# isl-org/adaptive-surface-reconstruction

Hardware: AMD Instinct MI355X
Metric: input points/sec to signed implicit values (higher is better)
Workload: dtype f32 via bf16x3 (24-bit operands, f32 accumulate)

## Files before the change

### adaptive-surface-reconstruction_amd/csrc/asr_api.hip

```cpp
#include <cmath>
#include <cstdlib>
#include <cstring>

#include <algorithm>
#include <functional>
#include <future>
#include <mutex>
#include <thread>

#include "asr_common.h"
#include "asr_uset.h"

#define ASR_ROW_GROUP_SEGMENT (ctx->opt.row_segment > 0 ? ctx->opt.row_segment : (i64)524288)
#define CTX_GUARD(ctx)                                                  \
    if (!(ctx)) return ASR_HIP_EINVAL;                                  \
    (ctx)->err.clear();                                                 \
    if (hipSetDevice((ctx)->device) != hipSuccess) {                    \
        (ctx)->err = "hipSetDevice failed for the context's device";   \
        return ASR_HIP_EHIP;                                            \
    }

namespace {
struct OptEntry {
    const char* name;
    const char* env;
    i64 AsrOptions::*field;
};
const OptEntry k_options[] = {
        {"sconv_min_blocks", "ASR_SCONV_MIN_BLOCKS", &AsrOptions::sconv_min_blocks},
        {"sconv_wide_min", "ASR_SCONV_WIDE_MIN", &AsrOptions::sconv_wide_min},
        {"row_segment", "ASR_ROW_SEGMENT", &AsrOptions::row_segment},
        {"row_lpt", "ASR_ROW_LPT", &AsrOptions::row_lpt},
        {"row_ranked", "ASR_ROW_RANKED", &AsrOptions::row_ranked},
        {"sconv_plan", "ASR_SCONV_PLAN", &AsrOptions::sconv_plan},
        {"plan_arena", "ASR_PLAN_ARENA", &AsrOptions::plan_arena},
        {"sconv16_min_blocks", "ASR_SCONV16_MIN_BLOCKS", &AsrOptions::sconv16_min_blocks},
        {"knn_cells", "ASR_KNN_CELLS", &AsrOptions::knn_cells},
        {"knn_deep", "ASR_KNN_DEEP", &AsrOptions::knn_deep},
        {"search_hash_level", "ASR_SEARCH_HASH_LEVEL", &AsrOptions::search_hash_level},
        {"overlap", "ASR_OVERLAP", &AsrOptions::overlap},
        {"build_search", "ASR_BUILD_SEARCH", &AsrOptions::build_search},
        {"cconv_valu", "ASR_CCONV_VALU", &AsrOptions::cconv_valu},
        {"search_half", "ASR_SEARCH_HALF", &AsrOptions::search_half},
        {"search_priority", "ASR_SEARCH_PRIORITY", &AsrOptions::search_priority},
        {"shard_timing", "ASR_SHARD_TIMING", &AsrOptions::shard_timing},
        {"shard_geometry", "ASR_SHARD_GEOMETRY", &AsrOptions::shard_geometry},
        {"early_sort", "ASR_EARLY_SORT", &AsrOptions::early_sort},
        {"early_cells", "ASR_EARLY_CELLS", &AsrOptions::early_cells},
        {"sconv_split_rows", "ASR_SCONV_SPLIT_ROWS", &AsrOptions::sconv_split_rows},
        {"sconv_split_min_rows", "ASR_SCONV_SPLIT_MIN_ROWS", &AsrOptions::sconv_split_min_rows},
        {"arena_cap_mb", "ASR_ARENA_CAP_MB", &AsrOptions::arena_cap_mb},
        {"inject_failure", "ASR_INJECT_FAILURE", &AsrOptions::inject_failure},
};
void apply_arena_cap(asr_hip_context* ctx) {
    const size_t cap = ctx->opt.arena_cap_mb > 0 ? (size_t)ctx->opt.arena_cap_mb << 20 : 0;
    for (asr_hip_context* c : {ctx, ctx->aux})
// ... 930 lines not shown
            const i64* rs;
            const int32_t* perm;
            i64 rows;
            int K;
        };
        std::vector<Job> jobs;
        for (int i = 0; i < ASR_NUM_GRIDS; ++i) {
            GridDev& g = ctx->grids[i];
            jobs.push_back({g.nidx, g.nkidx, g.nrs, g.perm_nb, g.v, 55});
            if (i + 1 < ASR_NUM_GRIDS) {
                GridDev& c = ctx->grids[i + 1];
                jobs.push_back({g.up_idx, g.up_kidx, g.up_rs, g.perm_up, g.v, 9});
                jobs.push_back({g.down_idx, g.down_kidx, g.down_rs, g.perm_down, c.v, 9});
            }
        }
        std::vector<asr_conv_plan> plans(jobs.size());
        for (size_t j = 0; j < jobs.size(); ++j) {
            plans[j].nidx = jobs[j].idx;
            plans[j].kidx = jobs[j].kidx;
            plans[j].rs = jobs[j].rs;
            plans[j].perm = jobs[j].perm;
            plans[j].num_out = jobs[j].rows;
            plans[j].K = jobs[j].K;
        }
        const int rc = asr_geom_conv_plan_batch(on, on->persist, plans.data(), (int)plans.size());
        if (rc != ASR_HIP_OK) {
            if (on != ctx) ctx->err = on->err;
            return rc;
        }
        for (size_t j = 0; j < jobs.size(); ++j) ctx->conv_plans[jobs[j].rs] = plans[j];
    }
    return ASR_HIP_OK;
}

__global__ void k_gather_queries(const int32_t* rows, i64 nq, const float* centers, const float* sizes, const u64* keys,
                                 float* qc, float* qs, u64* qk) {
    const i64 i = blockIdx.x * (i64)blockDim.x + threadIdx.x;
    if (i >= nq) return;
    const i64 r = rows[i];
    qc[3 * i] = centers[3 * r];
    qc[3 * i + 1] = centers[3 * r + 1];
    qc[3 * i + 2] = centers[3 * r + 2];
    qs[i] = sizes[r];
    qk[i] = keys[r];
}
__global__ void k_scatter_rows(const float* src, const int32_t* rows, i64 nq, int c, float* dst) {
// ... 667 lines not shown
```

### adaptive-surface-reconstruction_amd/csrc/asr_common.h

```cpp
#pragma once
#include <hip/hip_runtime.h>

#include <cstdint>
#include <cstdio>
#include <map>
#include <string>
#include <tuple>
#include <vector>

#include "../../include/asr_hip.h"

typedef uint64_t u64;
typedef int64_t i64;
typedef uint32_t u32;

struct Arena {
    struct Slab {
        char* base;
        size_t size, used;
    };
    std::vector<Slab> slabs;
    size_t min_slab = size_t(256) << 20;
    size_t cap = 0;

// ... 48 lines not shown
    i64* nrs = nullptr;
    int32_t* up_idx = nullptr;
    uint8_t* up_kidx = nullptr;
    i64* up_rs = nullptr;
    int32_t* down_idx = nullptr;
    uint8_t* down_kidx = nullptr;
    i64* down_rs = nullptr;
    int32_t* perm_nb = nullptr;
    int32_t* perm_up = nullptr;
    int32_t* perm_down = nullptr;
};

struct AsrOptions {
    i64 sconv_min_blocks = 2816;
    i64 sconv16_min_blocks = 1024;
    i64 sconv_wide_min = 2048;
    i64 row_segment = 524288;
    i64 search_hash_level = -1;
    i64 knn_deep = 1;
    i64 knn_cells = 1;
    i64 plan_arena = 0;
    i64 sconv_plan = 1;
    i64 row_ranked = 1;
    i64 row_lpt = 1;
    i64 overlap = 1;
    i64 cconv_valu = 0;
    i64 build_search = 1;
    i64 shard_geometry = -1;
    i64 shard_timing = 0;
    i64 search_priority = 2;
    i64 search_half = 1;
    i64 early_cells = 1;
    i64 early_sort = 1;
    i64 arena_cap_mb = 0;
    i64 inject_failure = 0;
    i64 sconv_split_min_rows = 2048;
    i64 sconv_split_rows = 32768;
};

struct asr_conv_plan_view {
    const uint4* hdr;
    const int32_t* pool;
    i64 groups;
    unsigned pool_bytes;
};
struct asr_conv_plan {
    uint4* hdr = nullptr;
    int32_t* pool = nullptr;
    i64 groups = 0, groups_pad = 0, blocks = 0;
    i64* offs = nullptr;
    const int32_t* nidx = nullptr;
    const uint8_t* kidx = nullptr;
    const i64* rs = nullptr;
    const int32_t* perm = nullptr;
    i64 num_out = 0;
    int K = 0;
    bool usable() const { return hdr && blocks * 64 < (i64(1) << 32) - 65536; }
    asr_conv_plan_view view() const { return {hdr, pool, groups, (unsigned)(blocks * 64)}; }
};

struct AsrPointIndex {
    bool valid = false;
    const float* pts = nullptr;
    const float* radii = nullptr;
    i64 n = 0;
    int lsort = 0;
    float4* sorted = nullptr;
    int32_t* ids = nullptr;
    int32_t* rank = nullptr;
    float* srad = nullptr;
    u64* codes = nullptr;
    u64* tab_keys = nullptr;
    u64 tab_mask = 0;
    int32_t* tab_start = nullptr;
    int32_t* tab_end = nullptr;
    int tab_lmin = 0, tab_lmax = -1, tab_lhash = 0, tab_grow = 0;
};

struct asr_hip_context {
// ... 214 lines not shown
int asr_geom_grid_neighbors_count(asr_hip_context* ctx, const u64* keys, i64 v, const int32_t* rows, i64 nrows, i64* rs,
                                  i64* num_pairs);
int asr_geom_grid_neighbors_fill(asr_hip_context* ctx, const u64* keys, i64 v, const int32_t* rows, i64 nrows,
                                 const i64* rs, int32_t* idx, uint8_t* kidx);
struct asr_nb_job {
    const u64* keys;
    i64 v;
    i64* rs;
    int32_t* idx;
    uint8_t* kidx;
    i64 p;
    const int32_t* owner = nullptr;
    int me = 0;
};
int asr_geom_neighbors_build_batch(asr_hip_context* ctx, Arena& out_arena, asr_nb_job* jobs, int n);
int asr_geom_row_groups(asr_hip_context* ctx, const uint8_t* kidx, const i64* rs, i64 v, i64 seg,
                        int32_t* perm_out, int kbits);
struct asr_row_group_job {
    const uint8_t* kidx;
    const i64* rs;
    i64 v;
    int kbits;
    int32_t* perm_out;
};
int asr_geom_row_groups_batch(asr_hip_context* ctx, const asr_row_group_job* jobs, int n, i64 seg);
int asr_geom_coarsen_count(asr_hip_context* ctx, const u64* keys, i64 v, i64* v_out);
int asr_geom_coarsen_fill(asr_hip_context* ctx, const u64* keys, i64 v, u64* out_keys, i64 v_out,
                          int32_t* up_idx, uint8_t* up_kidx, i64* up_rs);
int asr_geom_coarsen_build(asr_hip_context* ctx, Arena& keep, const u64* keys, i64 v, u64** out_keys, i64* v_out,
                           int32_t** up_idx, uint8_t** up_kidx, i64** up_rs, int32_t** down_idx, uint8_t** down_kidx,
                           i64** down_rs);
int asr_geom_voxel_info(asr_hip_context* ctx, const asr_octree_frame* frame, const u64* keys,
                        i64 v, float* centers, float* sizes);
int asr_geom_radius_count(asr_hip_context* ctx, const asr_octree_frame* frame, const float* pts,
                          i64 n, const float* centers, const float* sizes, i64 v, i64* rs,
                          i64* num_pairs, Arena* keep = nullptr, const float* radii = nullptr,
                          const u64* voxel_keys = nullptr, int lmin_hint = -1, int lmax_hint = -1,
                          const AsrPointIndex* pre = nullptr);

int asr_geom_radius_fill(asr_hip_context* ctx, const float* pts, const float* radii, i64 n,
                         const float* centers, const float* sizes, i64 v, const i64* rs,
                         int32_t* idx, float* dist, float* compat, int32_t* spos = nullptr,
                         const float4** sorted_out = nullptr);
int asr_geom_radius_neighbor_count(asr_hip_context* ctx, const asr_octree_frame* frame, const float* pts,
                                   const float* radii, i64 n, i64* counts_out);
int asr_geom_attributes_at(asr_hip_context* ctx, const asr_octree_frame* frame, const float* pts, const float* radii, i64 n,
                           const float* attr, int c, const float* positions, const float* sizes, i64 m, int max_widen,
                           float min_weight, float fill, float* out, float* weight_out, int8_t* widen_out);
// ... 60 lines not shown
```

### adaptive-surface-reconstruction_amd/csrc/asr_geom.hip

```cpp
#include <cstdlib>
#include <cstring>
#include <algorithm>
#include <rocprim/rocprim.hpp>

#include "asr_common.h"
#include "asr_prim.h"

namespace {
using namespace asr_prim;

constexpr int BLK = 256;

struct HashTab {
    u64* keys;
    int32_t* vals;
    u64 mask;
};

struct TabProbe {
    u64 bucket, step, low, bmask;
    __device__ inline u64 slot() const { return ((bucket & bmask) << 6) | low; }
    __device__ inline void next() { bucket += step; }
};
__device__ inline TabProbe tab_probe(const HashTab& t, u64 key) {
// ... 551 lines not shown
}
__global__ void k_iota64(i64* out, i64 n) {
    i64 i = blockIdx.x * (i64)blockDim.x + threadIdx.x;
    if (i < n) out[i] = i;
}

__global__ void k_voxel_info(asr_octree_frame f, const u64* keys, i64 v, float* centers,
                             float* sizes) {
    i64 i = blockIdx.x * (i64)blockDim.x + threadIdx.x;
    if (i >= v) return;
    int x, y, z, lev;
    asr_key_coord(keys[i], x, y, z, lev);
    int s = ASR_MAX_LEVEL - lev;
    double half = 0.5 * (double)(u64(1) << s);
    double vs = (double)f.voxel_size[ASR_MAX_LEVEL];
    if (centers) {
        centers[3 * i + 0] = (float)((((x << s) - f.offset[0]) + half) * vs);
        centers[3 * i + 1] = (float)((((y << s) - f.offset[1]) + half) * vs);
        centers[3 * i + 2] = (float)((((z << s) - f.offset[2]) + half) * vs);
    }
    if (sizes) sizes[i] = f.voxel_size[lev];
}

__global__ void k_point_codes(asr_octree_frame f, const float* pts, i64 n, u64* codes,
                              int32_t* ids, int* cnt) {
    i64 i = blockIdx.x * (i64)blockDim.x + threadIdx.x;
    if (i >= n) return;
    if (!(isfinite(pts[3 * i]) && isfinite(pts[3 * i + 1]) && isfinite(pts[3 * i + 2]))) cnt[11] = 1;
    int x, y, z;
    frame_coord(f, pts[3 * i], pts[3 * i + 1], pts[3 * i + 2], ASR_MAX_LEVEL, x, y, z);
    const int lim = (1 << ASR_MAX_LEVEL) - 1;
    x = min(max(x, 0), lim);
    y = min(max(y, 0), lim);
    z = min(max(z, 0), lim);
    codes[i] = asr_morton3d((u64)x, (u64)y, (u64)z);
    ids[i] = (int32_t)i;
}
__global__ void k_gather_points(const float* pts, const int32_t* ids, i64 n, float4* sorted, int32_t* rank,
                                const float* radii = nullptr, float* srad = nullptr) {
    i64 i = blockIdx.x * (i64)blockDim.x + threadIdx.x;
    if (i >= n) return;
    int32_t id = ids[i];
    sorted[i] = make_float4(pts[3 * (i64)id], pts[3 * (i64)id + 1], pts[3 * (i64)id + 2],
                            __int_as_float(id));
    if (rank) rank[id] = (int32_t)i;
    if (srad) srad[i] = radii[id];
}
__global__ void k_gather_radii(const float* radii, const int32_t* ids, i64 n, float* out) {
    i64 i = blockIdx.x * (i64)blockDim.x + threadIdx.x;
    if (i < n) out[i] = radii[ids[i]];
}
__device__ inline int query_level(const asr_octree_frame& f, float r) {
    int lev = 0;
    while (lev < ASR_MAX_LEVEL && f.voxel_size[lev + 1] >= r) ++lev;
    return lev;
}
__global__ __launch_bounds__(256) void k_query_levels(asr_octree_frame f, const float* sizes, i64 v, int* cnt) {
    __shared__ int s_lo[4], s_hi[4];
    int lo = ASR_MAX_LEVEL, hi = 0;
// ... 1171 lines not shown
        __syncthreads();
        const int m = min(2048, n - base);
        for (int e = 0; e < m; ++e) rank += s_key[e] < mine;
    }
    if (i < n) t.vals[slot_of[i]] = rank;
}
__global__ void k_rg_keys_ranked(RowGroupBatch b, i64 seg, const u64* masks, HashTab t, unsigned* keys, int32_t* ids,
                                 int rank_bits) {
    const i64 e = blockIdx.x * (i64)blockDim.x + threadIdx.x;
    if (e >= b.base[b.n]) return;
    const int j = rg_job_of(b, e);
    const i64 r = e - b.base[j];
    unsigned key;
    if (r < b.v[j]) {
        const int rank = tab_find(t, (masks[e] >> 1) + 1);
        key = ((unsigned)j << (6 + rank_bits)) | ((unsigned)(r / seg) << rank_bits) | (unsigned)rank;
    } else {
        key = ((unsigned)j << (6 + rank_bits)) | (63u << rank_bits) | ((1u << rank_bits) - 1u);
    }
    keys[e] = key;
    ids[e] = (int32_t)e;
}

__device__ inline u64 dev_morton_add(u64 a, u64 b) {
    const u64 M = 0x9249249249249249ull;
    u64 c = ((a | ~M) + (b & M)) & M;
    c |= ((a | ~(M << 1)) + (b & (M << 1))) & (M << 1);
    c |= ((a | ~(M << 2)) + (b & (M << 2))) & (M << 2);
    return c;
}
__device__ inline u64 dev_morton_sub(u64 a, u64 b) {
    const u64 M = 0x9249249249249249ull;
    u64 c = ((a & M) - (b & M)) & M;
    c |= ((a & (M << 1)) - (b & (M << 1))) & (M << 1);
    c |= ((a & (M << 2)) - (b & (M << 2))) & (M << 2);
    return c;
}
__device__ inline int node_lookup(const HashTab& t, u64 key) {
    TabProbe pr = tab_probe(t, key);
    for (u64 probe = 0; probe <= pr.bmask; ++probe, pr.next()) {
        const u64 slot = pr.slot();
        const u64 cur = t.keys[slot];
        if (cur == key) return t.vals[slot];
        if (cur == 0) return -2;
    }
    return -2;
// ... 412 lines not shown
    }
    if (perm_m != perm_out) {
        const i64 nc = (v + 127) / 128;
        int32_t* ckey = arena_alloc<int32_t>(ctx->scratch, nc);
        int32_t* ckey_s = arena_alloc<int32_t>(ctx->scratch, nc);
        int32_t* cid = arena_alloc<int32_t>(ctx->scratch, nc);
        int32_t* cid_s = arena_alloc<int32_t>(ctx->scratch, nc);
        if (!ckey || !ckey_s || !cid || !cid_s) ASR_FAIL(ctx, ASR_HIP_EHIP, "arena allocation failed");
        int32_t* tcost = arena_alloc<int32_t>(ctx->scratch, 2 * nc);
        if (!tcost) ASR_FAIL(ctx, ASR_HIP_EHIP, "arena allocation failed");
        k_tile_cost<<<grid_for(((v + 63) / 64) * 64, BLK), BLK, 0, ctx->stream>>>(perm_m, masks, v, tcost);
        ASR_CHECK_LAUNCH(ctx);
        k_chunk_key<<<grid_for(nc, BLK), BLK, 0, ctx->stream>>>(tcost, v, seg, ckey, cid);
        ASR_CHECK_LAUNCH(ctx);
        ASR_TRY((sort_pairs<int32_t, int32_t>(ctx, ctx->scratch, ckey, ckey_s, cid, cid_s, nc,
                                              7 + bits_for((v + seg - 1) / seg + 1))));
        k_chunk_apply<<<grid_for(v, BLK), BLK, 0, ctx->stream>>>(perm_m, cid_s, v, perm_out);
        ASR_CHECK_LAUNCH(ctx);
    }
    return ASR_HIP_OK;
}

static int rg_batch_run(asr_hip_context* ctx, const asr_row_group_job* jobs, int n, i64 seg, int mask_bits);
static int rg_batch_run_ranked(asr_hip_context* ctx, const asr_row_group_job* jobs, int n, i64 seg, bool* done);
int asr_geom_row_groups_batch(asr_hip_context* ctx, const asr_row_group_job* jobs, int n, i64 seg) {
    if (seg < 128) seg = 128;
    bool fits = n <= RG_MAX_JOBS && seg % 128 == 0;
    for (int j = 0; j < n && fits; ++j) fits = jobs[j].v / seg < 63 && jobs[j].v < (i64(1) << 31);
    if (!fits) {
        for (int j = 0; j < n; ++j)
            ASR_TRY(asr_geom_row_groups(ctx, jobs[j].kidx, jobs[j].rs, jobs[j].v, seg, jobs[j].perm_out, jobs[j].kbits));
        return ASR_HIP_OK;
    }
    if (ctx->opt.row_ranked) {
        bool done = false;
        ASR_TRY(rg_batch_run_ranked(ctx, jobs, n, seg, &done));
        if (done) return ASR_HIP_OK;
    }
    std::vector<asr_row_group_job> small_jobs, wide_jobs;
    for (int j = 0; j < n; ++j) (jobs[j].kbits <= 10 ? small_jobs : wide_jobs).push_back(jobs[j]);
    if (!small_jobs.empty()) ASR_TRY(rg_batch_run(ctx, small_jobs.data(), (int)small_jobs.size(), seg, 9));
    if (!wide_jobs.empty()) ASR_TRY(rg_batch_run(ctx, wide_jobs.data(), (int)wide_jobs.size(), seg, 54));
    return ASR_HIP_OK;
}
static int rg_batch_run_ranked(asr_hip_context* ctx, const asr_row_group_job* jobs, int n, i64 seg, bool* done) {
    *done = false;
    ASR_TRY(ensure_flags(ctx));
    RowGroupBatch b;
    b.n = 0;
    i64 total = 0;
    for (int j = 0; j < n; ++j) {
        if (jobs[j].v <= 0) continue;
        b.base[b.n] = total;
        b.v[b.n] = jobs[j].v;
        b.kidx[b.n] = jobs[j].kidx;
        b.rs[b.n] = jobs[j].rs;
        b.out[b.n] = jobs[j].perm_out;
        total += (jobs[j].v + 127) / 128 * 128;
        ++b.n;
    }
    if (b.n == 0) {
        *done = true;
        return ASR_HIP_OK;
    }
    b.base[b.n] = total;
    if (total >= (i64(1) << 31)) ASR_FAIL(ctx, ASR_HIP_EINVAL, "row_groups: too many rows");
    u64* masks = arena_alloc<u64>(ctx->scratch, total);
    unsigned* keys = arena_alloc<unsigned>(ctx->scratch, total);
// ... 5 lines not shown
    int32_t* ckey_s = arena_alloc<int32_t>(ctx->scratch, nc);
    int32_t* cid = arena_alloc<int32_t>(ctx->scratch, nc);
    int32_t* cid_s = arena_alloc<int32_t>(ctx->scratch, nc);
    if (!masks || !keys || !keys_s || !ids || !ids_s || !ckey || !ckey_s || !cid || !cid_s)
        ASR_FAIL(ctx, ASR_HIP_EHIP, "arena allocation failed");
    HashTab t;
    ASR_TRY(make_table(ctx, ctx->scratch, RG_MASK_TAB, true, t));
    ASR_TRY(fresh_flags(ctx));
    k_rg_masks<<<grid_for(total, BLK), BLK, 0, ctx->stream>>>(b, masks, t, ctx->d_flags);
    ASR_CHECK_LAUNCH(ctx);
    u64* mlist = arena_alloc<u64>(ctx->scratch, RG_MAX_MASKS);
    int32_t* mslot = arena_alloc<int32_t>(ctx->scratch, RG_MAX_MASKS);
    if (!mlist || !mslot) ASR_FAIL(ctx, ASR_HIP_EHIP, "arena allocation failed");
    k_rg_mask_collect<<<grid_for((i64)t.mask + 1, BLK), BLK, 0, ctx->stream>>>(t, mlist, mslot, ctx->d_flags);
    ASR_CHECK_LAUNCH(ctx);
    k_rg_mask_ranks<<<RG_MAX_MASKS / 256, 256, 0, ctx->stream>>>(t, mlist, mslot, ctx->d_flags);
    ASR_CHECK_LAUNCH(ctx);
    int host[16];
    ASR_TRY(read_flags(ctx, host));
    if (host[1] || host[2] > RG_MAX_MASKS) return ASR_HIP_OK;
    const int rank_bits = bits_for(std::max(host[2], 2));
    k_rg_keys_ranked<<<grid_for(total, BLK), BLK, 0, ctx->stream>>>(b, seg, masks, t, keys, ids, rank_bits);
    ASR_CHECK_LAUNCH(ctx);
    ASR_TRY((sort_pairs<unsigned, int32_t>(ctx, ctx->scratch, keys, keys_s, ids, ids_s, total, 4 + 6 + rank_bits)));
    const int lpt = ctx->opt.row_lpt != 0;
    if (lpt) {
        k_rg_chunk_keys<<<grid_for(nc * 64, BLK), BLK, 0, ctx->stream>>>(b, seg, ids_s, masks, ckey, cid);
        ASR_CHECK_LAUNCH(ctx);
        ASR_TRY((sort_pairs<int32_t, int32_t>(ctx, ctx->scratch, ckey, ckey_s, cid, cid_s, nc, 17)));
    }
    k_rg_apply<<<grid_for(total, BLK), BLK, 0, ctx->stream>>>(b, ids_s, cid_s, lpt);
    ASR_CHECK_LAUNCH(ctx);
    *done = true;
    return ASR_HIP_OK;
}
static int rg_batch_run(asr_hip_context* ctx, const asr_row_group_job* jobs, int n, i64 seg, int mask_bits) {
    RowGroupBatch b;
    b.n = 0;
    i64 total = 0;
    for (int j = 0; j < n; ++j) {
        if (jobs[j].v <= 0) continue;
        b.base[b.n] = total;
        b.v[b.n] = jobs[j].v;
        b.kidx[b.n] = jobs[j].kidx;
        b.rs[b.n] = jobs[j].rs;
        b.out[b.n] = jobs[j].perm_out;
        total += (jobs[j].v + 127) / 128 * 128;
        ++b.n;
    }
    if (b.n == 0) return ASR_HIP_OK;
    b.base[b.n] = total;
    if (total >= (i64(1) << 31)) ASR_FAIL(ctx, ASR_HIP_EINVAL, "row_groups: too many rows");
    u64* keys = arena_alloc<u64>(ctx->scratch, total);
    u64* keys_s = arena_alloc<u64>(ctx->scratch, total);
    u64* masks = arena_alloc<u64>(ctx->scratch, total);
// ... 131 lines not shown
    i64 num_heavy = 0;
    int* hc_pref = nullptr;
    int* hc_beg = nullptr;
    const u64* dual_leaves = nullptr;
    i64 dual_nl = 0;
    float* srad = nullptr;
    const float* radii_src = nullptr;
    int lsort = 0;
    int cell_grow = 0;
    bool aligned = false;
    bool aligned_main = false;
    AlignedQ aq = {nullptr, nullptr, nullptr, -1};
};
static RadiusState& rstate(asr_hip_context* ctx) {
    if (!ctx->radius_state) ctx->radius_state = new RadiusState();
    return *(RadiusState*)ctx->radius_state;
}
void asr_geom_release(asr_hip_context* ctx) {
    delete (RadiusState*)ctx->radius_state;
    ctx->radius_state = nullptr;
}

static int sort_points(asr_hip_context* ctx, const asr_octree_frame* frame, const float* pts, i64 n, int lsort,
                       RadiusState& st, Arena* keep, bool want_rank, const float* radii, bool keep_all = false) {
    st.frame = *frame;
    st.n = n;
    st.lsort = lsort;
    Arena& ka = keep ? *keep : ctx->scratch;
    u64* codes_u = arena_alloc<u64>(ctx->scratch, n + 1);
    u64* codes = arena_alloc<u64>(keep_all ? ka : ctx->scratch, n + 1);
    int32_t* ids_u = arena_alloc<int32_t>(ctx->scratch, n + 1);
    int32_t* ids = arena_alloc<int32_t>(ka, n + 1);
    st.sorted = arena_alloc<float4>(ka, n + 1);
    st.ids = ids;
    st.codes = codes;
    st.codes_w = codes;
    st.codes_u = codes_u;
    st.ids_u = ids_u;
    st.ids_w = ids;
    st.rank = want_rank ? arena_alloc<int32_t>(ka, n + 1) : nullptr;
    st.srad = radii ? arena_alloc<float>(keep_all ? ka : ctx->scratch, n + 1) : nullptr;
    st.radii_src = radii;
    if (!codes_u || !codes || !ids_u || !ids || !st.sorted || (want_rank && !st.rank) || (radii && !st.srad))
        ASR_FAIL(ctx, ASR_HIP_EHIP, "arena allocation failed");
    if (n > 0) {
        k_point_codes<<<grid_for(n, BLK), BLK, 0, ctx->stream>>>(*frame, pts, n, codes_u, ids_u, ctx->d_flags);
        ASR_CHECK_LAUNCH(ctx);
        ASR_TRY((sort_pairs<u64, int32_t>(ctx, ctx->scratch, codes_u, codes, ids_u, ids, n, 63,
                                          3 * (ASR_MAX_LEVEL - std::max(lsort, 1)))));
        k_gather_points<<<grid_for(n, BLK), BLK, 0, ctx->stream>>>(pts, ids, n, st.sorted, st.rank, radii, st.srad);
        ASR_CHECK_LAUNCH(ctx);
    }
    return ASR_HIP_OK;
}
static int build_cell_table(asr_hip_context* ctx, i64 n, int lmin, int lmax, RadiusState& st, bool hash_all,
                            Arena* where = nullptr);
static int build_point_index(asr_hip_context* ctx, const asr_octree_frame* frame, const float* pts,
                             i64 n, int lmin, int lmax, RadiusState& st, Arena* keep = nullptr,
                             bool want_rank = false, bool hash_all = true, const float* radii = nullptr) {
    ASR_TRY(fresh_flags(ctx));
    ASR_TRY(sort_points(ctx, frame, pts, n, lmax, st, keep, want_rank, radii));
    return build_cell_table(ctx, n, lmin, lmax, st, hash_all);
}
static int build_cell_table(asr_hip_context* ctx, i64 n, int lmin, int lmax, RadiusState& st, bool hash_all, Arena* where) {
    Arena& arena = where ? *where : ctx->scratch;
    int host[16];
    const u64* codes = st.codes;
    HashTab dummy{nullptr, nullptr, 0};
    int* level_cnt = ctx->d_flags + 32;
    int host_lvl[ASR_MAX_LEVEL + 1] = {0};
// ... 9 lines not shown
    int lhash = lmax;
    if (!hash_all) {
        lhash = lmin;
        while (lhash < lmax && (i64)host_lvl[lhash + 1] * 2 <= n) ++lhash;
        if (ctx->opt.search_hash_level >= 0) lhash = (int)std::min<i64>(lmax, std::max<i64>(lmin - 1, ctx->opt.search_hash_level));
    }
    st.lhash = lhash;
    i64 cells = 0;
    for (int l = lmin; l <= lhash; ++l) cells += host_lvl[l];
    u64 cap = next_pow2((u64)std::max<i64>(1024, 2 * cells)) << st.cell_grow;
    ASR_TRY(make_table(ctx, arena, cap, false, st.tab));
    st.start = arena_alloc<int32_t>(arena, cap);
    st.end = arena_alloc<int32_t>(arena, cap);
    if (!st.start || !st.end) ASR_FAIL(ctx, ASR_HIP_EHIP, "arena allocation failed");
    if (n > 0) {
        k_cell_bounds<false><<<grid_for(n + 1, BLK), BLK, 0, ctx->stream>>>(
                codes, n, lmin, lhash, st.tab, st.start, st.end, ctx->d_flags, nullptr);
        ASR_CHECK_LAUNCH(ctx);
    }
    return ASR_HIP_OK;
}

constexpr int PRESORT_LEVEL = 13;
__global__ __launch_bounds__(256) void k_finest_point_level(asr_octree_frame f, const float* __restrict__ radii, i64 n,
                                                            float radius_scale, int max_depth, int* __restrict__ out) {
    int m = 0;
    for (i64 i = blockIdx.x * (i64)blockDim.x + threadIdx.x; i < n; i += (i64)gridDim.x * blockDim.x) {
        int l = level_from_scale(f, radius_scale * radii[i]);
        l = l < max_depth ? l : max_depth;
        m = max(m, l);
    }
#pragma unroll
    for (int o = 32; o > 0; o >>= 1) m = max(m, __shfl_xor(m, o, 64));
    if ((threadIdx.x & 63) == 0 && m > 0) atomicMax(out, m);
}
int asr_geom_presort(asr_hip_context* ctx, Arena& keep, const asr_octree_frame* frame, const float* pts,
                     const float* radii, i64 n, float radius_scale, int max_depth) {
    ASR_TRY(ensure_flags(ctx));
    AsrPointIndex& pi = ctx->pindex;
    pi.valid = false;
    if (n <= 0 || n >= (i64(1) << 31)) return ASR_HIP_OK;
    int lsort = PRESORT_LEVEL;
    if (radius_scale > 0.f && radii) {
        int host[16];
        ASR_TRY(fresh_flags(ctx));
        k_finest_point_level<<<std::min<unsigned>(grid_for(n, BLK), 2048u), BLK, 0, ctx->stream>>>(
                *frame, radii, n, radius_scale, std::min(max_depth, ASR_MAX_LEVEL), ctx->d_flags + 8);
        ASR_CHECK_LAUNCH(ctx);
        ASR_TRY(read_flags(ctx, host));
        lsort = std::max(PRESORT_LEVEL, std::min(ASR_MAX_LEVEL, host[8] + 1));
    }
    RadiusState st;
    ASR_TRY(sort_points(ctx, frame, pts, n, lsort, st, &keep, true, radii, true));
    pi.pts = pts;
    pi.radii = radii;
    pi.n = n;
    pi.lsort = lsort;
    pi.sorted = st.sorted;
    pi.ids = st.ids;
    pi.rank = st.rank;
    pi.srad = st.srad;
    pi.codes = st.codes_w;
    pi.valid = true;
    return ASR_HIP_OK;
}

int asr_geom_precells(asr_hip_context* ctx, Arena& keep) {
    AsrPointIndex& pi = ctx->pindex;
    pi.tab_keys = nullptr;
    if (!pi.valid || pi.n <= 0) return ASR_HIP_OK;
    RadiusState st;
    st.codes = st.codes_w = pi.codes;
    st.n = pi.n;
    st.cell_grow = rstate(ctx).cell_grow;
    ASR_TRY(fresh_flags(ctx));
    ASR_TRY(build_cell_table(ctx, pi.n, 1, pi.lsort, st, false, &keep));
// ... 527 lines not shown
    if (plan->num_out <= 0) return ASR_HIP_OK;
    plan->blocks = blocks;
    plan->pool = (int32_t*)keep.alloc((size_t)(blocks > 0 ? blocks : 1) * 64);
    if (!plan->pool) ASR_FAIL(ctx, ASR_HIP_EHIP, "arena allocation failed");
    ASR_HIP_CHECK(ctx, hipMemsetAsync(plan->pool, 0xFF, (size_t)(blocks > 0 ? blocks : 1) * 64, ctx->stream));
    k_plan_fill<<<grid_for(plan->groups_pad * 16, BLK), BLK, 0, ctx->stream>>>(
            plan->nidx, plan->kidx, plan->rs, plan->perm, plan->num_out, plan->K, plan->groups_pad, plan->offs,
            plan->hdr, plan->pool);
    ASR_CHECK_LAUNCH(ctx);
    return ASR_HIP_OK;
}

namespace {
constexpr int PLAN_MAX_JOBS = 16;
struct PlanBatch {
    int n;
    i64 base[PLAN_MAX_JOBS + 1];
    i64 rows[PLAN_MAX_JOBS];
    int K[PLAN_MAX_JOBS];
    const int32_t* nidx[PLAN_MAX_JOBS];
    const uint8_t* kidx[PLAN_MAX_JOBS];
    const i64* rs[PLAN_MAX_JOBS];
    const int32_t* perm[PLAN_MAX_JOBS];
};
__device__ inline int plan_job_of(const PlanBatch& b, i64 row) {
    int j = 0;
    while (j + 1 < b.n && row >= b.base[j + 1]) ++j;
    return j;
}
__global__ void k_plan_masks_batch(PlanBatch b, uint4* __restrict__ hdr, i64* __restrict__ counts) {
    const i64 grow = blockIdx.x * (i64)blockDim.x + threadIdx.x;
    if (grow >= b.base[b.n]) return;
    const int j = plan_job_of(b, grow);
    const i64 row = grow - b.base[j];
    unsigned long long m = 0;
    if (row < b.rows[j]) {
        const i64 q = b.perm[j] ? b.perm[j][row] : row;
        const uint8_t* kidx = b.kidx[j];
        for (i64 p = b.rs[j][q], pe = b.rs[j][q + 1]; p < pe; ++p) {
            const int k = kidx[p];
            if (k < b.K[j]) m |= 1ull << k;
        }
    }
#pragma unroll
    for (int o = 1; o < 16; o <<= 1) m |= __shfl_xor(m, o, 64);
    if ((threadIdx.x & 15) == 0) {
        hdr[grow >> 4] = make_uint4((unsigned)m, (unsigned)(m >> 32), 0u, 0u);
        counts[grow >> 4] = (i64)__popcll(m);
    }
}
__global__ void k_plan_fill_batch(PlanBatch b, const i64* __restrict__ offs, uint4* __restrict__ hdr,
                                  int32_t* __restrict__ pool) {
    const i64 grow = blockIdx.x * (i64)blockDim.x + threadIdx.x;
    if (grow >= b.base[b.n]) return;
    const i64 grp = grow >> 4;
    const unsigned off = (unsigned)offs[grp];
    if ((grow & 15) == 0) hdr[grp].z = off;
    const int j = plan_job_of(b, grow);
    const i64 row = grow - b.base[j];
    const uint2 h = *reinterpret_cast<const uint2*>(&hdr[grp]);
    unsigned long long m = (unsigned long long)h.x | ((unsigned long long)h.y << 32);
    i64 p = 0, pe = 0;
    const uint8_t* kidx = b.kidx[j];
    const int32_t* nidx = b.nidx[j];
    if (row < b.rows[j]) {
        const i64 q = b.perm[j] ? b.perm[j][row] : row;
        p = b.rs[j][q];
        pe = b.rs[j][q + 1];
    }
    int32_t* line = pool + (i64)off * 16 + (grow & 15);
    while (m) {
        const int k = __builtin_ctzll(m);
        m &= m - 1;
        while (p < pe && kidx[p] < k) ++p;
        int32_t v = -1;
        if (p < pe && kidx[p] == k) v = nidx[p++];
        *line = v;
        line += 16;
    }
}
}

int asr_geom_conv_plan_batch(asr_hip_context* ctx, Arena& keep, asr_conv_plan* plans, int n) {
    if (n > PLAN_MAX_JOBS) ASR_FAIL(ctx, ASR_HIP_EINVAL, "conv_plan_batch: too many lists");
    PlanBatch b;
    memset(&b, 0, sizeof(b));
    b.n = 0;
    i64 total = 0;
    int which[PLAN_MAX_JOBS];
    for (int j = 0; j < n; ++j) {
        asr_conv_plan& pl = plans[j];
        pl.hdr = nullptr;
        pl.pool = nullptr;
        pl.offs = nullptr;
        pl.groups = pl.groups_pad = pl.blocks = 0;
        if (pl.num_out <= 0) continue;
        pl.groups = (pl.num_out + 15) / 16;
        pl.groups_pad = (pl.groups + 15) / 16 * 16;
        which[b.n] = j;
        b.base[b.n] = total;
        b.rows[b.n] = pl.num_out;
        b.K[b.n] = pl.K;
        b.nidx[b.n] = pl.nidx;
        b.kidx[b.n] = pl.kidx;
        b.rs[b.n] = pl.rs;
        b.perm[b.n] = pl.perm;
        total += pl.groups_pad * 16;
        ++b.n;
    }
    b.base[b.n] = total;
    if (b.n == 0) return ASR_HIP_OK;
    const i64 groups = total / 16;
    uint4* hdr = (uint4*)keep.alloc(groups * sizeof(uint4));
    i64* offs = (i64*)keep.alloc((groups + 1) * sizeof(i64));
    i64* counts = (i64*)ctx->scratch.alloc((groups + 1) * sizeof(i64));
    if (!hdr || !offs || !counts) ASR_FAIL(ctx, ASR_HIP_EHIP, "arena allocation failed");
    ASR_HIP_CHECK(ctx, hipMemsetAsync(counts + groups, 0, sizeof(i64), ctx->stream));
    k_plan_masks_batch<<<grid_for(total, BLK), BLK, 0, ctx->stream>>>(b, hdr, counts);
    ASR_CHECK_LAUNCH(ctx);
    ASR_TRY(asr_prim::scan_counts(ctx, ctx->scratch, counts, offs, groups + 1));
    i64 blocks = 0;
    ASR_TRY(asr_prim::read_i64(ctx, offs + groups, &blocks));
    int32_t* pool = (int32_t*)keep.alloc((size_t)(blocks > 0 ? blocks : 1) * 64);
    if (!pool) ASR_FAIL(ctx, ASR_HIP_EHIP, "arena allocation failed");
    k_plan_fill_batch<<<grid_for(total, BLK), BLK, 0, ctx->stream>>>(b, offs, hdr, pool);
    ASR_CHECK_LAUNCH(ctx);
    for (int t = 0; t < b.n; ++t) {
        asr_conv_plan& pl = plans[which[t]];
        pl.hdr = hdr + b.base[t] / 16;
// ... 20 lines not shown
```

Before: 276.5 million.

## Add custom radix sort for row groups, reuse row masks in plan build, fuse finest-level scan

Adds a custom 8-bit-digit radix sort (histogram plus scatter kernels using wave ballot matching) for the row-group key sort, enabled by default through a new row_sort option. Row-group occupancy masks are handed to conv plan building so the per-row mask no longer has to be rebuilt from kidx scans. The plan fill kernel now finds neighbor indices by popcount on the row mask instead of a linear merge, processing four entries at a time. The finest-point-level reduction is folded into the point-codes kernel, removing a separate pass over the radii. The hand-written sort may be slower than rocprim's for some sizes, and the masks approach assumes the kidx values in each row are sorted and unique.

Measured after the change: 278.7 million (median of 3 runs). About the same (+0.8%).

```diff
diff --git a/adaptive-surface-reconstruction_amd/csrc/asr_api.hip b/adaptive-surface-reconstruction_amd/csrc/asr_api.hip
--- a/adaptive-surface-reconstruction_amd/csrc/asr_api.hip
+++ b/adaptive-surface-reconstruction_amd/csrc/asr_api.hip
@@ -32,6 +32,7 @@
         {"row_segment", "ASR_ROW_SEGMENT", &AsrOptions::row_segment},
         {"row_lpt", "ASR_ROW_LPT", &AsrOptions::row_lpt},
         {"row_ranked", "ASR_ROW_RANKED", &AsrOptions::row_ranked},
+        {"row_sort", "ASR_ROW_SORT", &AsrOptions::row_sort},
         {"sconv_plan", "ASR_SCONV_PLAN", &AsrOptions::sconv_plan},
         {"plan_arena", "ASR_PLAN_ARENA", &AsrOptions::plan_arena},
         {"sconv16_min_blocks", "ASR_SCONV16_MIN_BLOCKS", &AsrOptions::sconv16_min_blocks},
@@ -1008,6 +1009,8 @@
             plans[j].perm = jobs[j].perm;
             plans[j].num_out = jobs[j].rows;
             plans[j].K = jobs[j].K;
+            for (const asr_row_group_job& r : rg_jobs)
+                if (r.rs == jobs[j].rs) plans[j].masks = r.masks;
         }
         const int rc = asr_geom_conv_plan_batch(on, on->persist, plans.data(), (int)plans.size());
         if (rc != ASR_HIP_OK) {
diff --git a/adaptive-surface-reconstruction_amd/csrc/asr_common.h b/adaptive-surface-reconstruction_amd/csrc/asr_common.h
--- a/adaptive-surface-reconstruction_amd/csrc/asr_common.h
+++ b/adaptive-surface-reconstruction_amd/csrc/asr_common.h
@@ -94,6 +94,7 @@
     i64 plan_arena = 0;
     i64 sconv_plan = 1;
     i64 row_ranked = 1;
+    i64 row_sort = 1;
     i64 row_lpt = 1;
     i64 overlap = 1;
     i64 cconv_valu = 0;
@@ -127,6 +128,7 @@
     const int32_t* perm = nullptr;
     i64 num_out = 0;
     int K = 0;
+    const u64* masks = nullptr;
     bool usable() const { return hdr && blocks * 64 < (i64(1) << 32) - 65536; }
     asr_conv_plan_view view() const { return {hdr, pool, groups, (unsigned)(blocks * 64)}; }
 };
@@ -387,8 +389,9 @@
     i64 v;
     int kbits;
     int32_t* perm_out;
-};
-int asr_geom_row_groups_batch(asr_hip_context* ctx, const asr_row_group_job* jobs, int n, i64 seg);
+    const u64* masks = nullptr;
+};
+int asr_geom_row_groups_batch(asr_hip_context* ctx, asr_row_group_job* jobs, int n, i64 seg);
 int asr_geom_coarsen_count(asr_hip_context* ctx, const u64* keys, i64 v, i64* v_out);
 int asr_geom_coarsen_fill(asr_hip_context* ctx, const u64* keys, i64 v, u64* out_keys, i64 v_out,
                           int32_t* up_idx, uint8_t* up_kidx, i64* up_rs);
diff --git a/adaptive-surface-reconstruction_amd/csrc/asr_geom.hip b/adaptive-surface-reconstruction_amd/csrc/asr_geom.hip
--- a/adaptive-surface-reconstruction_amd/csrc/asr_geom.hip
+++ b/adaptive-surface-reconstruction_amd/csrc/asr_geom.hip
@@ -597,19 +597,36 @@
     if (sizes) sizes[i] = f.voxel_size[lev];
 }
 
-__global__ void k_point_codes(asr_octree_frame f, const float* pts, i64 n, u64* codes,
-                              int32_t* ids, int* cnt) {
+__global__ __launch_bounds__(BLK) void k_point_codes(asr_octree_frame f, const float* pts, i64 n, u64* codes, int32_t* ids,
+                                                     int* cnt, const float* __restrict__ radii = nullptr,
+                                                     float radius_scale = 0.f, int max_depth = 0) {
+    __shared__ int s_lvl[BLK / 64];
     i64 i = blockIdx.x * (i64)blockDim.x + threadIdx.x;
-    if (i >= n) return;
-    if (!(isfinite(pts[3 * i]) && isfinite(pts[3 * i + 1]) && isfinite(pts[3 * i + 2]))) cnt[11] = 1;
-    int x, y, z;
-    frame_coord(f, pts[3 * i], pts[3 * i + 1], pts[3 * i + 2], ASR_MAX_LEVEL, x, y, z);
-    const int lim = (1 << ASR_MAX_LEVEL) - 1;
-    x = min(max(x, 0), lim);
-    y = min(max(y, 0), lim);
-    z = min(max(z, 0), lim);
-    codes[i] = asr_morton3d((u64)x, (u64)y, (u64)z);
-    ids[i] = (int32_t)i;
+    if (i < n) {
+        if (!(isfinite(pts[3 * i]) && isfinite(pts[3 * i + 1]) && isfinite(pts[3 * i + 2]))) cnt[11] = 1;
+        int x, y, z;
+        frame_coord(f, pts[3 * i], pts[3 * i + 1], pts[3 * i + 2], ASR_MAX_LEVEL, x, y, z);
+        const int lim = (1 << ASR_MAX_LEVEL) - 1;
+        x = min(max(x, 0), lim);
+        y = min(max(y, 0), lim);
+        z = min(max(z, 0), lim);
+        codes[i] = asr_morton3d((u64)x, (u64)y, (u64)z);
+        ids[i] = (int32_t)i;
+    }
+    if (!radii) return;
+    int m = 0;
+    if (i < n) {
+        m = level_from_scale(f, radius_scale * radii[i]);
+        m = m < max_depth ? m : max_depth;
+    }
+#pragma unroll
+    for (int o = 32; o > 0; o >>= 1) m = max(m, __shfl_xor(m, o, 64));
+    if ((threadIdx.x & 63) == 0) s_lvl[threadIdx.x >> 6] = m;
+    __syncthreads();
+    if (threadIdx.x == 0) {
+        for (int w = 1; w < BLK / 64; ++w) m = max(m, s_lvl[w]);
+        if (m > 0) atomicMax(cnt + 8, m);
+    }
 }
 __global__ void k_gather_points(const float* pts, const int32_t* ids, i64 n, float4* sorted, int32_t* rank,
                                 const float* radii = nullptr, float* srad = nullptr) {
@@ -1827,6 +1844,93 @@
     ids[e] = (int32_t)e;
 }
 
+constexpr int RS_ITEMS = 16;
+constexpr int RS_TILE = BLK * RS_ITEMS;
+constexpr int RS_DIGITS = 256;
+static_assert(BLK == RS_DIGITS, "thread d of a block owns digit d of its tile");
+__device__ inline u64 rs_match(unsigned d, u64 valid) {
+    u64 m = valid;
+#pragma unroll
+    for (int b = 0; b < 8; ++b) {
+        const u64 bal = __ballot((d >> b) & 1u);
+        m &= ((d >> b) & 1u) ? bal : ~bal;
+    }
+    return m;
+}
+__global__ __launch_bounds__(BLK) void k_rs_hist(const unsigned* __restrict__ keys, i64 n, int shift, int ntiles,
+                                                 int* __restrict__ counts) {
+    __shared__ int s_h[BLK / 64][RS_DIGITS];
+    const int lane = threadIdx.x & 63, wave = threadIdx.x >> 6;
+    for (int w = 0; w < BLK / 64; ++w) s_h[w][threadIdx.x] = 0;
+    __syncthreads();
+    volatile int* h = s_h[wave];
+    const i64 first = (i64)blockIdx.x * RS_TILE + (i64)wave * (64 * RS_ITEMS) + lane;
+    unsigned key[RS_ITEMS];
+#pragma unroll
+    for (int r = 0; r < RS_ITEMS; ++r) key[r] = first + r * 64 < n ? keys[first + r * 64] : 0u;
+#pragma unroll
+    for (int r = 0; r < RS_ITEMS; ++r) {
+        const bool valid = first + r * 64 < n;
+        const unsigned d = (key[r] >> shift) & (RS_DIGITS - 1);
+        const u64 m = rs_match(d, __ballot(valid));
+        if (valid && (m & ((u64(1) << lane) - 1)) == 0) h[d] += __popcll(m);
+        __builtin_amdgcn_wave_barrier();
+    }
+    __syncthreads();
+    int c = 0;
+    for (int w = 0; w < BLK / 64; ++w) c += s_h[w][threadIdx.x];
+    counts[(i64)threadIdx.x * ntiles + blockIdx.x] = c;
+}
+__global__ __launch_bounds__(BLK) void k_rs_scatter(const unsigned* __restrict__ kin, const int32_t* __restrict__ vin, i64 n,
+                                                    int shift, int ntiles, const int* __restrict__ offs,
+                                                    unsigned* __restrict__ kout, int32_t* __restrict__ vout) {
+    __shared__ int s_h[BLK / 64][RS_DIGITS];
+    const int lane = threadIdx.x & 63, wave = threadIdx.x >> 6;
+    for (int w = 0; w < BLK / 64; ++w) s_h[w][threadIdx.x] = 0;
+    __syncthreads();
+    volatile int* h = s_h[wave];
+    const i64 first = (i64)blockIdx.x * RS_TILE + (i64)wave * (64 * RS_ITEMS) + lane;
+    unsigned key[RS_ITEMS];
+    int32_t val[RS_ITEMS];
+    int rank[RS_ITEMS];
+#pragma unroll
+    for (int r = 0; r < RS_ITEMS; ++r) {
+        const bool valid = first + r * 64 < n;
+        key[r] = valid ? kin[first + r * 64] : 0u;
+        val[r] = valid ? vin[first + r * 64] : 0;
+    }
+#pragma unroll
+    for (int r = 0; r < RS_ITEMS; ++r) {
+        const bool valid = first + r * 64 < n;
+        const unsigned d = (key[r] >> shift) & (RS_DIGITS - 1);
+        const u64 m = rs_match(d, __ballot(valid));
+        const u64 below = m & ((u64(1) << lane) - 1);
+        const int before = h[d];
+        rank[r] = before + __popcll(below);
+        __builtin_amdgcn_wave_barrier();
+        if (valid && below == 0) h[d] = before + __popcll(m);
+        __builtin_amdgcn_wave_barrier();
+    }
+    __syncthreads();
+    {
+        int o = offs[(i64)threadIdx.x * ntiles + blockIdx.x];
+        for (int w = 0; w < BLK / 64; ++w) {
+            const int c = s_h[w][threadIdx.x];
+            s_h[w][threadIdx.x] = o;
+            o += c;
+        }
+    }
+    __syncthreads();
+#pragma unroll
+    for (int r = 0; r < RS_ITEMS; ++r) {
+        if (first + r * 64 >= n) continue;
+        const i64 pos = (i64)s_h[wave][(key[r] >> shift) & (RS_DIGITS - 1)] + rank[r];
+        if (pos < 0 || pos >= n) continue;
+        if (kout) kout[pos] = key[r];
+        vout[pos] = val[r];
+    }
+}
+
 __device__ inline u64 dev_morton_add(u64 a, u64 b) {
     const u64 M = 0x9249249249249249ull;
     u64 c = ((a | ~M) + (b & M)) & M;
@@ -2285,8 +2389,9 @@
 }
 
 static int rg_batch_run(asr_hip_context* ctx, const asr_row_group_job* jobs, int n, i64 seg, int mask_bits);
-static int rg_batch_run_ranked(asr_hip_context* ctx, const asr_row_group_job* jobs, int n, i64 seg, bool* done);
-int asr_geom_row_groups_batch(asr_hip_context* ctx, const asr_row_group_job* jobs, int n, i64 seg) {
+static int rg_batch_run_ranked(asr_hip_context* ctx, asr_row_group_job* jobs, int n, i64 seg, bool* done);
+int asr_geom_row_groups_batch(asr_hip_context* ctx, asr_row_group_job* jobs, int n, i64 seg) {
+    for (int j = 0; j < n; ++j) jobs[j].masks = nullptr;
     if (seg < 128) seg = 128;
     bool fits = n <= RG_MAX_JOBS && seg % 128 == 0;
     for (int j = 0; j < n && fits; ++j) fits = jobs[j].v / seg < 63 && jobs[j].v < (i64(1) << 31);
@@ -2306,7 +2411,37 @@
     if (!wide_jobs.empty()) ASR_TRY(rg_batch_run(ctx, wide_jobs.data(), (int)wide_jobs.size(), seg, 54));
     return ASR_HIP_OK;
 }
-static int rg_batch_run_ranked(asr_hip_context* ctx, const asr_row_group_job* jobs, int n, i64 seg, bool* done) {
+static int rs_sort_pairs(asr_hip_context* ctx, Arena& arena, const unsigned* kin, unsigned* kout, const int32_t* vin,
+                         int32_t* vout, i64 n, int end_bit) {
+    if (n <= 0) return ASR_HIP_OK;
+    const int passes = std::max(1, (end_bit + 7) / 8);
+    const int ntiles = (int)((n + RS_TILE - 1) / RS_TILE);
+    const size_t table = (size_t)RS_DIGITS * ntiles;
+    int* counts = arena_alloc<int>(arena, table);
+    int* offs = arena_alloc<int>(arena, table);
+    unsigned* ktmp = passes > 1 ? arena_alloc<unsigned>(arena, n) : nullptr;
+    int32_t* vtmp = passes > 1 ? arena_alloc<int32_t>(arena, n) : nullptr;
+    size_t tb = 0;
+    ASR_HIP_CHECK(ctx, rocprim::exclusive_scan(nullptr, tb, counts, offs, 0, table, rocprim::plus<int>(), ctx->stream));
+    void* tmp = arena.alloc(tb ? tb : 256);
+    if (!counts || !offs || !tmp || (passes > 1 && (!ktmp || !vtmp))) ASR_FAIL(ctx, ASR_HIP_EHIP, "arena allocation failed");
+    const unsigned* ksrc = kin;
+    const int32_t* vsrc = vin;
+    for (int p = 0; p < passes; ++p) {
+        const bool to_out = (passes - 1 - p) % 2 == 0;
+        unsigned* kdst = p == passes - 1 ? nullptr : (to_out ? kout : ktmp);
+        int32_t* vdst = to_out ? vout : vtmp;
+        k_rs_hist<<<ntiles, BLK, 0, ctx->stream>>>(ksrc, n, 8 * p, ntiles, counts);
+        ASR_CHECK_LAUNCH(ctx);
+        ASR_HIP_CHECK(ctx, rocprim::exclusive_scan(tmp, tb, counts, offs, 0, table, rocprim::plus<int>(), ctx->stream));
+        k_rs_scatter<<<ntiles, BLK, 0, ctx->stream>>>(ksrc, vsrc, n, 8 * p, ntiles, offs, kdst, vdst);
+        ASR_CHECK_LAUNCH(ctx);
+        ksrc = kdst;
+        vsrc = vdst;
+    }
+    return ASR_HIP_OK;
+}
+static int rg_batch_run_ranked(asr_hip_context* ctx, asr_row_group_job* jobs, int n, i64 seg, bool* done) {
     *done = false;
     ASR_TRY(ensure_flags(ctx));
     RowGroupBatch b;
@@ -2358,7 +2493,10 @@
     const int rank_bits = bits_for(std::max(host[2], 2));
     k_rg_keys_ranked<<<grid_for(total, BLK), BLK, 0, ctx->stream>>>(b, seg, masks, t, keys, ids, rank_bits);
     ASR_CHECK_LAUNCH(ctx);
-    ASR_TRY((sort_pairs<unsigned, int32_t>(ctx, ctx->scratch, keys, keys_s, ids, ids_s, total, 4 + 6 + rank_bits)));
+    if (ctx->opt.row_sort)
+        ASR_TRY(rs_sort_pairs(ctx, ctx->scratch, keys, keys_s, ids, ids_s, total, 4 + 6 + rank_bits));
+    else
+        ASR_TRY((sort_pairs<unsigned, int32_t>(ctx, ctx->scratch, keys, keys_s, ids, ids_s, total, 4 + 6 + rank_bits)));
     const int lpt = ctx->opt.row_lpt != 0;
     if (lpt) {
         k_rg_chunk_keys<<<grid_for(nc * 64, BLK), BLK, 0, ctx->stream>>>(b, seg, ids_s, masks, ckey, cid);
@@ -2367,6 +2505,8 @@
     }
     k_rg_apply<<<grid_for(total, BLK), BLK, 0, ctx->stream>>>(b, ids_s, cid_s, lpt);
     ASR_CHECK_LAUNCH(ctx);
+    for (int j = 0, t = 0; j < n; ++j)
+        if (jobs[j].v > 0) jobs[j].masks = masks + b.base[t++];
     *done = true;
     return ASR_HIP_OK;
 }
@@ -2544,7 +2684,8 @@
 }
 
 static int sort_points(asr_hip_context* ctx, const asr_octree_frame* frame, const float* pts, i64 n, int lsort,
-                       RadiusState& st, Arena* keep, bool want_rank, const float* radii, bool keep_all = false) {
+                       RadiusState& st, Arena* keep, bool want_rank, const float* radii, bool keep_all = false,
+                       float finest_scale = 0.f, int finest_cap = 0) {
     st.frame = *frame;
     st.n = n;
     st.lsort = lsort;
@@ -2566,8 +2707,15 @@
     if (!codes_u || !codes || !ids_u || !ids || !st.sorted || (want_rank && !st.rank) || (radii && !st.srad))
         ASR_FAIL(ctx, ASR_HIP_EHIP, "arena allocation failed");
     if (n > 0) {
-        k_point_codes<<<grid_for(n, BLK), BLK, 0, ctx->stream>>>(*frame, pts, n, codes_u, ids_u, ctx->d_flags);
+        const bool finest = radii && finest_scale > 0.f;
+        k_point_codes<<<grid_for(n, BLK), BLK, 0, ctx->stream>>>(*frame, pts, n, codes_u, ids_u, ctx->d_flags,
+                                                                 finest ? radii : nullptr, finest_scale, finest_cap);
         ASR_CHECK_LAUNCH(ctx);
+        if (finest) {
+            int host[16];
+            ASR_TRY(read_flags(ctx, host));
+            st.lsort = lsort = std::max(lsort, std::min(ASR_MAX_LEVEL, host[8] + 1));
+        }
         ASR_TRY((sort_pairs<u64, int32_t>(ctx, ctx->scratch, codes_u, codes, ids_u, ids, n, 63,
                                           3 * (ASR_MAX_LEVEL - std::max(lsort, 1)))));
         k_gather_points<<<grid_for(n, BLK), BLK, 0, ctx->stream>>>(pts, ids, n, st.sorted, st.rank, radii, st.srad);
@@ -2623,36 +2771,18 @@
 }
 
 constexpr int PRESORT_LEVEL = 13;
-__global__ __launch_bounds__(256) void k_finest_point_level(asr_octree_frame f, const float* __restrict__ radii, i64 n,
-                                                            float radius_scale, int max_depth, int* __restrict__ out) {
-    int m = 0;
-    for (i64 i = blockIdx.x * (i64)blockDim.x + threadIdx.x; i < n; i += (i64)gridDim.x * blockDim.x) {
-        int l = level_from_scale(f, radius_scale * radii[i]);
-        l = l < max_depth ? l : max_depth;
-        m = max(m, l);
-    }
-#pragma unroll
-    for (int o = 32; o > 0; o >>= 1) m = max(m, __shfl_xor(m, o, 64));
-    if ((threadIdx.x & 63) == 0 && m > 0) atomicMax(out, m);
-}
 int asr_geom_presort(asr_hip_context* ctx, Arena& keep, const asr_octree_frame* frame, const float* pts,
                      const float* radii, i64 n, float radius_scale, int max_depth) {
     ASR_TRY(ensure_flags(ctx));
     AsrPointIndex& pi = ctx->pindex;
     pi.valid = false;
     if (n <= 0 || n >= (i64(1) << 31)) return ASR_HIP_OK;
-    int lsort = PRESORT_LEVEL;
-    if (radius_scale > 0.f && radii) {
-        int host[16];
-        ASR_TRY(fresh_flags(ctx));
-        k_finest_point_level<<<std::min<unsigned>(grid_for(n, BLK), 2048u), BLK, 0, ctx->stream>>>(
-                *frame, radii, n, radius_scale, std::min(max_depth, ASR_MAX_LEVEL), ctx->d_flags + 8);
-        ASR_CHECK_LAUNCH(ctx);
-        ASR_TRY(read_flags(ctx, host));
-        lsort = std::max(PRESORT_LEVEL, std::min(ASR_MAX_LEVEL, host[8] + 1));
-    }
+    const bool finest = radius_scale > 0.f && radii;
+    if (finest) ASR_TRY(fresh_flags(ctx));
     RadiusState st;
-    ASR_TRY(sort_points(ctx, frame, pts, n, lsort, st, &keep, true, radii, true));
+    ASR_TRY(sort_points(ctx, frame, pts, n, PRESORT_LEVEL, st, &keep, true, radii, true, finest ? radius_scale : 0.f,
+                        std::min(max_depth, ASR_MAX_LEVEL)));
+    const int lsort = st.lsort;
     pi.pts = pts;
     pi.radii = radii;
     pi.n = n;
@@ -3226,11 +3356,23 @@
     const uint8_t* kidx[PLAN_MAX_JOBS];
     const i64* rs[PLAN_MAX_JOBS];
     const int32_t* perm[PLAN_MAX_JOBS];
+    const u64* masks[PLAN_MAX_JOBS];
 };
 __device__ inline int plan_job_of(const PlanBatch& b, i64 row) {
     int j = 0;
     while (j + 1 < b.n && row >= b.base[j + 1]) ++j;
     return j;
+}
+__device__ inline u64 plan_row_mask(const PlanBatch& b, int j, i64 q, i64 p, i64 pe) {
+    const u64 kmask = b.K[j] >= 64 ? ~u64(0) : (u64(1) << b.K[j]) - 1;
+    if (b.masks[j]) return b.masks[j][q] & kmask;
+    const uint8_t* kidx = b.kidx[j];
+    u64 m = 0;
+    for (; p < pe; ++p) {
+        const int k = kidx[p];
+        if (k < 64) m |= u64(1) << k;
+    }
+    return m & kmask;
 }
 __global__ void k_plan_masks_batch(PlanBatch b, uint4* __restrict__ hdr, i64* __restrict__ counts) {
     const i64 grow = blockIdx.x * (i64)blockDim.x + threadIdx.x;
@@ -3240,11 +3382,8 @@
     unsigned long long m = 0;
     if (row < b.rows[j]) {
         const i64 q = b.perm[j] ? b.perm[j][row] : row;
-        const uint8_t* kidx = b.kidx[j];
-        for (i64 p = b.rs[j][q], pe = b.rs[j][q + 1]; p < pe; ++p) {
-            const int k = kidx[p];
-            if (k < b.K[j]) m |= 1ull << k;
-        }
+        if (b.masks[j]) m = plan_row_mask(b, j, q, 0, 0);
+        else m = plan_row_mask(b, j, q, b.rs[j][q], b.rs[j][q + 1]);
     }
 #pragma unroll
     for (int o = 1; o < 16; o <<= 1) m |= __shfl_xor(m, o, 64);
@@ -3264,23 +3403,34 @@
     const i64 row = grow - b.base[j];
     const uint2 h = *reinterpret_cast<const uint2*>(&hdr[grp]);
     unsigned long long m = (unsigned long long)h.x | ((unsigned long long)h.y << 32);
-    i64 p = 0, pe = 0;
-    const uint8_t* kidx = b.kidx[j];
-    const int32_t* nidx = b.nidx[j];
+    i64 p = 0;
+    u64 rm = 0;
+    const int32_t* __restrict__ nidx = b.nidx[j];
     if (row < b.rows[j]) {
         const i64 q = b.perm[j] ? b.perm[j][row] : row;
         p = b.rs[j][q];
-        pe = b.rs[j][q + 1];
+        rm = plan_row_mask(b, j, q, p, b.rs[j][q + 1]);
     }
     int32_t* line = pool + (i64)off * 16 + (grow & 15);
     while (m) {
-        const int k = __builtin_ctzll(m);
-        m &= m - 1;
-        while (p < pe && kidx[p] < k) ++p;
-        int32_t v = -1;
-        if (p < pe && kidx[p] == k) v = nidx[p++];
-        *line = v;
-        line += 16;
+        int k[4];
+        int32_t v[4];
+#pragma unroll
+        for (int t = 0; t < 4; ++t) {
+            k[t] = m ? __builtin_ctzll(m) : -1;
+            m &= m - 1;
+        }
+#pragma unroll
+        for (int t = 0; t < 4; ++t) {
+            v[t] = -1;
+            if (k[t] >= 0 && ((rm >> k[t]) & 1)) v[t] = nidx[p + __popcll(rm & ((u64(1) << k[t]) - 1))];
+        }
+#pragma unroll
+        for (int t = 0; t < 4; ++t)
+            if (k[t] >= 0) {
+                *line = v[t];
+                line += 16;
+            }
     }
 }
 }
@@ -3309,6 +3459,8 @@
         b.kidx[b.n] = pl.kidx;
         b.rs[b.n] = pl.rs;
         b.perm[b.n] = pl.perm;
+        b.masks[b.n] = pl.masks;
+        pl.masks = nullptr;
         total += pl.groups_pad * 16;
         ++b.n;
     }
```
